# Meowuu7/equi-articulated-pose

Measured on AMD Instinct MI355X. Metric: point-clouds/sec (4096 pts, 60 anchors) fwd+bwd, higher is better.
Workload: dtype f32; 1 GPU; 8 x 4096-pt synthetic laptop clouds per GPU, 3-block inter backbone 1->64->128->512 (NN=64,K=24,A=60), forward+backward+Adam; clouds_per_gpu=8, points=4096, anchors=60

## Files before the change

### equi-articulated-pose_amd/csrc/so3_dense.hip

```cpp
#include <atomic>
#include "common.h"
#include "device_prims.h"
#include <type_traits>

namespace {

typedef unsigned long long u64;
typedef const __attribute__((address_space(4))) unsigned long long *cu64p;

constexpr int KC_BK = 32;
constexpr int KC_LIST_BYTES = 4096;

__host__ __device__ __forceinline__ void dense_kr(int d, int ks, int &k, int &r) {
    const int g = d / (16 * ks), rem = d - g * 16 * ks;
    k = rem >> 4;
    r = 16 * g + (rem & 15);
}


__device__ __forceinline__ void split2(float x0, float x1, unsigned &h, unsigned &l) {
    asm("v_cvt_pk_f16_f32 %0, %2, %3\n\t"
        "v_fma_mixlo_f16 %1, %0, -1.0, %2 op_sel:[0,0,0] op_sel_hi:[1,0,0]\n\t"
        "v_fma_mixhi_f16 %1, %0, -1.0, %3 op_sel:[1,0,0] op_sel_hi:[1,0,0]"
        : "=&v"(h), "=&v"(l) : "v"(x0), "v"(x1));
// ... 175 lines not shown
__global__ __launch_bounds__(256) void dense_rows_kernel(int n_sup, int na, int ks, int rp, int kd_pad, int rows_ld,
                                                         const float *__restrict__ s_xyz, const float *__restrict__ centre,
                                                         const int32_t *__restrict__ rows, const float *__restrict__ rk,
                                                         const float *__restrict__ row_rot, f32x4 *__restrict__ kr) {
    const int b = blockIdx.z, a = blockIdx.y, i = blockIdx.x * 256 + threadIdx.x;
    if (i >= kd_pad) return;
    f32x4 v = {1e4f, 1e4f, 1e4f, 0.f};
    if (i < ks * rp) {
        int k, r;
        dense_kr(i, ks, k, r);
        const int row = rows[(size_t)b * rows_ld + r];
        if ((unsigned)row < (unsigned)n_sup) {
            const float *kp = rk + ((size_t)a * ks + k) * 3;
            double k0 = (double)kp[0], k1 = (double)kp[1], k2 = (double)kp[2];
            if (row_rot != nullptr) {
                const float *M = row_rot + ((size_t)b * rows_ld + r) * 9;
                const double t0 = M[0] * k0 + M[1] * k1 + M[2] * k2, t1 = M[3] * k0 + M[4] * k1 + M[5] * k2, t2 = M[6] * k0 + M[7] * k1 + M[8] * k2;
                k0 = t0; k1 = t1; k2 = t2;
            }
            const double x = (double)s_xyz[((size_t)b * 3 + 0) * n_sup + row] - (double)centre[b * 4 + 0] - k0;
            const double y = (double)s_xyz[((size_t)b * 3 + 1) * n_sup + row] - (double)centre[b * 4 + 1] - k1;
            const double z = (double)s_xyz[((size_t)b * 3 + 2) * n_sup + row] - (double)centre[b * 4 + 2] - k2;
            v = (f32x4){(float)x, (float)y, (float)z, 0.f};
        }
    }
    kr[((size_t)b * na + a) * kd_pad + i] = v;
}

__global__ __launch_bounds__(256) void dense_rowmax_kernel(int m, int l, int na, int seg, long long seg_pitch4, const int32_t *__restrict__ colmap,
                                                           const f32x4 *__restrict__ T, float *__restrict__ scale, float *__restrict__ scale2) {
    __shared__ unsigned s[256][4];
    const int nq = na >> 2, G = 256 / nq, b = blockIdx.y, row = blockIdx.x, t = threadIdx.x;
    const int aq = t % nq, pg = t / nq;
    unsigned v0 = 0, v1 = 0, v2 = 0, v3 = 0;
    if (pg < G) {
        const f32x4 *src = T + ((size_t)b * m + row) * (colmap ? (size_t)1 : (size_t)(l / seg)) * seg_pitch4;
        for (int i0 = pg; i0 < l; i0 += 8 * G) {
            f32x4 q[8];
#pragma unroll
            for (int u = 0; u < 8; ++u) {
                const int i = min(i0 + u * G, l - 1), sg = i / seg;
                if (colmap != nullptr) {
                    const int ci = colmap[(size_t)b * l + i];
                    q[u] = ci >= 0 ? src[(size_t)ci * nq + aq] : (f32x4){0.f, 0.f, 0.f, 0.f};
                } else {
                    q[u] = src[(size_t)sg * seg_pitch4 + (size_t)(i - sg * seg) * nq + aq];
                }
            }
#pragma unroll
            for (int u = 0; u < 8; ++u) {
                v0 = max(v0, __float_as_uint(q[u].x) & 0x7fffffffu);
                v1 = max(v1, __float_as_uint(q[u].y) & 0x7fffffffu);
                v2 = max(v2, __float_as_uint(q[u].z) & 0x7fffffffu);
                v3 = max(v3, __float_as_uint(q[u].w) & 0x7fffffffu);
            }
        }
    }
    s[t][0] = v0; s[t][1] = v1; s[t][2] = v2; s[t][3] = v3;
    __syncthreads();
    if (t < na) {
        unsigned v = 0;
        for (int g = 0; g < G; ++g) v = max(v, s[g * nq + (t >> 2)][t & 3]);
        const float sc = pow2_scale(__uint_as_float(v));
        scale[((size_t)b * na + t) * m + row] = sc;
        scale2[((size_t)b * m + row) * na + t] = sc;
    }
}

__global__ __launch_bounds__(256) void dense_scale_kernel(long long total, int m, int na, const unsigned *__restrict__ rowmax,
                                                          float *__restrict__ scale, float *__restrict__ scale2) {
    const long long i = (long long)blockIdx.x * 256 + threadIdx.x;
    if (i >= total) return;
    const int a = (int)(i % na);
    const long long br = i / na;
    const int row = (int)(br % m);
    const long long b = br / m;
    const float sc = pow2_scale(__uint_as_float(rowmax[i]));
    scale[(b * na + a) * m + row] = sc;
    scale2[i] = sc;
}

struct SplitBn { const f32x4 *Y2; const float *coef; float slope, inv_slope; };
template <bool BN>
__global__ __launch_bounds__(256) void dense_split_kernel(int nb, int m, int l, int na, int kb_total, int seg, long long seg_pitch4, int mapped,
                                                          const int32_t *__restrict__ n_rows, const int32_t *__restrict__ colmap,
                                                          const f32x4 *__restrict__ T, const float *__restrict__ scale2,
                                                          u32x4 *__restrict__ planes, SplitBn bn) {
    const int t = threadIdx.x;
    const int mts = m >> 5;
    const int kb = (int)(blockIdx.x % (unsigned)kb_total), grp_ = (int)(blockIdx.x / (unsigned)kb_total), mt = grp_ % mts, b = grp_ / mts;
    (void)nb;
    const int nq = na >> 2, RG = 256 / nq;
    const int aq = t % nq, rr = t / nq;
    if (rr >= RG) return;
    const int MT = m >> 5, nseg = l / seg;
    if (mapped && n_rows != nullptr && 16 * kb >= ((min(n_rows[b], seg) + 15) & ~15) * nseg) return;
    for (int it0 = rr; it0 < 64; it0 += 2 * RG) {
        f32x4 q[2][8];
        f32x4 q2[BN ? 2 : 1][BN ? 8 : 1];
        int rowv[2], lanef[2];
#pragma unroll
        for (int u = 0; u < 2; ++u) {
            const int it = min(it0 + u * RG, 63);
            const int i = it & 31, kg = it >> 5, row = 32 * mt + i, l0 = 16 * kb + 8 * kg;
            rowv[u] = row; lanef[u] = i + 32 * kg;
            const size_t row_off = ((size_t)b * m + row) * (colmap ? (size_t)1 : (size_t)nseg) * seg_pitch4 + aq;
            const f32x4 *src = T + row_off;
            int sg = l0 / seg, sr = l0 - sg * seg;
            if (mapped) dense_kr(l0, nseg, sg, sr);
            if (colmap != nullptr) {
                int ci[8] = {-1, -1, -1, -1, -1, -1, -1, -1};
                if (l0 < l) {
                    const int4 c0 = *reinterpret_cast<const int4 *>(colmap + (size_t)b * l + l0), c1 = *reinterpret_cast<const int4 *>(colmap + (size_t)b * l + l0 + 4);
                    ci[0] = c0.x; ci[1] = c0.y; ci[2] = c0.z; ci[3] = c0.w; ci[4] = c1.x; ci[5] = c1.y; ci[6] = c1.z; ci[7] = c1.w;
                }
#pragma unroll
                for (int e = 0; e < 8; ++e) q[u][e] = ci[e] >= 0 ? src[(size_t)ci[e] * nq] : (f32x4){0.f, 0.f, 0.f, 0.f};
                if constexpr (BN) {
#pragma unroll
                    for (int e = 0; e < 8; ++e) q2[u][e] = ci[e] >= 0 ? bn.Y2[row_off + (size_t)ci[e] * nq] : (f32x4){0.f, 0.f, 0.f, 0.f};
                }
            } else {
#pragma unroll
                for (int e = 0; e < 8; ++e) {
                    const bool in = l0 + e < l;
                    const size_t at = (size_t)sg * seg_pitch4 + (size_t)sr * nq;
                    q[u][e] = in ? src[at] : (f32x4){0.f, 0.f, 0.f, 0.f};
                    if constexpr (BN) q2[u][e] = in ? bn.Y2[row_off + at] : (f32x4){0.f, 0.f, 0.f, 0.f};
                    if (++sr == seg) { sr = 0; ++sg; }
                }
            }
        }
        if constexpr (BN) {
#pragma unroll
            for (int u = 0; u < 2; ++u) {
                const int it = min(it0 + u * RG, 63);
                const int l0 = 16 * kb + 8 * (it >> 5);
                const float k1 = bn.coef[rowv[u]], k2 = bn.coef[m + rowv[u]], k3 = bn.coef[2 * m + rowv[u]], be = bn.coef[3 * m + rowv[u]], ig = bn.coef[4 * m + rowv[u]];
                int live = 0;
                if (colmap != nullptr) {
                    if (l0 < l) {
                        const int4 c0 = *reinterpret_cast<const int4 *>(colmap + (size_t)b * l + l0), c1 = *reinterpret_cast<const int4 *>(colmap + (size_t)b * l + l0 + 4);
                        live = (c0.x >= 0) | (c0.y >= 0) << 1 | (c0.z >= 0) << 2 | (c0.w >= 0) << 3 | (c1.x >= 0) << 4 | (c1.y >= 0) << 5 | (c1.z >= 0) << 6 | (c1.w >= 0) << 7;
                    }
                } else {
                    for (int e = 0; e < 8; ++e) live |= (l0 + e < l) << e;
                }
#pragma unroll
                for (int e = 0; e < 8; ++e)
#pragma unroll
                    for (int j = 0; j < 4; ++j) {
                        const float yv = q2[u][e][j], gv = q[u][e][j];
                        const bool pos = yv > 0.f;
                        const float gg = pos ? gv : gv * bn.slope, pre = pos ? yv : yv * bn.inv_slope;
                        const float gx = fmaf(gg, k1, -k2) - ((pre - be) * ig) * k3;
                        q[u][e][j] = ((live >> e) & 1) ? gx : 0.f;
                    }
            }
        }
#pragma unroll
        for (int u = 0; u < 2; ++u) {
            if (it0 + u * RG >= 64) break;
            const f32x4 sc = *reinterpret_cast<const f32x4 *>(scale2 + ((size_t)b * m + rowv[u]) * na + 4 * aq);
#pragma unroll
            for (int j = 0; j < 4; ++j) {
                unsigned h[4], lo[4];
#pragma unroll
                for (int e = 0; e < 4; ++e) split2(q[u][2 * e][j] * sc[j], q[u][2 * e + 1][j] * sc[j], h[e], lo[e]);
                u32x4 *dst = planes + ((((size_t)b * na + 4 * aq + j) * kb_total + kb) * MT + mt) * 128 + lanef[u];
                dst[0] = (u32x4){h[0], h[1], h[2], h[3]};
                dst[64] = (u32x4){lo[0], lo[1], lo[2], lo[3]};
            }
        }
    }
}

template <int CSTEPS>
__global__ __launch_bounds__(256) void dense_gplanes_kernel(int m, int na, int ks, int rp, int rch, int kb_total, const float *__restrict__ W3,
                                                            const float *__restrict__ Ft, const int32_t *__restrict__ n_rows,
                                                            const float *__restrict__ bound, float *__restrict__ scale, u32x4 *__restrict__ planes) {
    constexpr int C = 16 * CSTEPS, PITCH = 2 * C + 16;
    extern __shared__ __attribute__((aligned(16))) unsigned char smem[];
    __shared__ unsigned s_red[4];
    const int z = blockIdx.y, b = z / na;
    const int t = threadIdx.x, lane = t & 63, li = lane & 31, kg = lane >> 5, wave = t >> 6;
    const int rows_b = n_rows ? min((min(n_rows[b], rp) + 15) & ~15, rp) : rp;
    unsigned char *Fh = smem, *Fl = smem + (size_t)rch * PITCH;
    const int MT = m >> 5, mt = blockIdx.x * 4 + wave;
    const bool active = mt < MT;
    const int o = 32 * min(mt, MT - 1) + li;
    const float s_out = pow2_scale(bound[(size_t)z * m + o]);
    if (active && kg == 0) scale[(size_t)z * m + o] = s_out;
    for (int rc0 = 0; rc0 < rows_b; rc0 += rch) {
        const int nrows = min(rch, rows_b - rc0);
        if (rc0 > 0) __syncthreads();
        const f32x4 *src = reinterpret_cast<const f32x4 *>(Ft + ((size_t)z * rp + rc0) * C);
        const int n4 = nrows * (C / 4);
        unsigned mx = 0;
        for (int i = t; i < n4; i += 256) {
            const f32x4 v = src[i];
            mx = max(mx, max(max(__float_as_uint(v.x) & 0x7fffffffu, __float_as_uint(v.y) & 0x7fffffffu),
                             max(__float_as_uint(v.z) & 0x7fffffffu, __float_as_uint(v.w) & 0x7fffffffu)));
        }
#pragma unroll
        for (int o_ = 32; o_ > 0; o_ >>= 1) mx = max(mx, (unsigned)__shfl_xor((int)mx, o_));
        if (lane == 0) s_red[wave] = mx;
        __syncthreads();
        const float sF = pow2_scale(__uint_as_float(max(max(s_red[0], s_red[1]), max(s_red[2], s_red[3]))));
        for (int i = t; i < n4; i += 256) {
            const f32x4 v = src[i];
            const int r = i / (C / 4), c4 = i - r * (C / 4);
            unsigned h0, l0, h1, l1;
            split2(v.x * sF, v.y * sF, h0, l0);
            split2(v.z * sF, v.w * sF, h1, l1);
            *reinterpret_cast<uint2 *>(Fh + (size_t)r * PITCH + c4 * 8) = make_uint2(h0, h1);
            *reinterpret_cast<uint2 *>(Fl + (size_t)r * PITCH + c4 * 8) = make_uint2(l0, l1);
        }
        __syncthreads();
        if (!active) continue;
        const int rtiles = (nrows + 31) >> 5;
        f32x4 wn[CSTEPS][2];
        auto load_w = [&](int k) __attribute__((always_inline)) {
            const f32x4 *wrow = reinterpret_cast<const f32x4 *>(W3 + ((size_t)o * ks + k) * C) + 2 * kg;
#pragma unroll
            for (int s_ = 0; s_ < CSTEPS; ++s_) { wn[s_][0] = wrow[4 * s_]; wn[s_][1] = wrow[4 * s_ + 1]; }
        };
        load_w(0);
        for (int k = 0; k < ks; ++k) {
            f32x4 w[CSTEPS][2];
            unsigned wm = 0;
#pragma unroll
            for (int s_ = 0; s_ < CSTEPS; ++s_) {
                w[s_][0] = wn[s_][0]; w[s_][1] = wn[s_][1];
#pragma unroll
                for (int e = 0; e < 4; ++e) wm = max(wm, max(__float_as_uint(w[s_][0][e]) & 0x7fffffffu, __float_as_uint(w[s_][1][e]) & 0x7fffffffu));
            }
            if (k + 1 < ks) load_w(k + 1);
            wm = max(wm, (unsigned)__shfl_xor((int)wm, 32));
            const float sW = pow2_scale(__uint_as_float(wm));
            u32x4 Bh[CSTEPS], Bl[CSTEPS];
#pragma unroll
            for (int s_ = 0; s_ < CSTEPS; ++s_) {
                unsigned h[4], l[4];
                split2(w[s_][0].x * sW, w[s_][0].y * sW, h[0], l[0]);
                split2(w[s_][0].z * sW, w[s_][0].w * sW, h[1], l[1]);
                split2(w[s_][1].x * sW, w[s_][1].y * sW, h[2], l[2]);
                split2(w[s_][1].z * sW, w[s_][1].w * sW, h[3], l[3]);
                Bh[s_] = (u32x4){h[0], h[1], h[2], h[3]};
                Bl[s_] = (u32x4){l[0], l[1], l[2], l[3]};
            }
            const float tsc = s_out / (sF * sW);
            for (int rt = 0; rt < rtiles; ++rt) {
                f32x16 acc;
#pragma unroll
                for (int i = 0; i < 16; ++i) acc[i] = 0.f;
                const int r = min(32 * rt + li, rch - 1);
                const unsigned char *ah = Fh + (size_t)r * PITCH + 16 * kg, *al = Fl + (size_t)r * PITCH + 16 * kg;
#pragma unroll
                for (int s_ = 0; s_ < CSTEPS; ++s_) {
                    const u32x4 fh = *reinterpret_cast<const u32x4 *>(ah + 32 * s_), fl = *reinterpret_cast<const u32x4 *>(al + 32 * s_);
                    acc = __builtin_amdgcn_mfma_f32_32x32x16_f16(__builtin_bit_cast(f16x8, fh), __builtin_bit_cast(f16x8, Bh[s_]), acc, 0, 0, 0);
                    acc = __builtin_amdgcn_mfma_f32_32x32x16_f16(__builtin_bit_cast(f16x8, fh), __builtin_bit_cast(f16x8, Bl[s_]), acc, 0, 0, 0);
                    acc = __builtin_amdgcn_mfma_f32_32x32x16_f16(__builtin_bit_cast(f16x8, fl), __builtin_bit_cast(f16x8, Bh[s_]), acc, 0, 0, 0);
                }
                float av[16];
#pragma unroll
                for (int i = 0; i < 16; ++i) { av[i] = acc[i]; asm volatile("" : "+v"(av[i])); }
                const bool hi = kg != 0;
                float snd[8], rcv[8];
#pragma unroll
                for (int e = 0; e < 4; ++e) { snd[e] = hi ? av[e] : av[4 + e]; snd[4 + e] = hi ? av[8 + e] : av[12 + e]; }
#pragma unroll
                for (int e = 0; e < 8; ++e) rcv[e] = __shfl_xor(snd[e], 32);
#pragma unroll
                for (int half = 0; half < 2; ++half) {
                    float v[8];
#pragma unroll
                    for (int e = 0; e < 4; ++e) {
                        const float own = (hi ? av[4 + 8 * half + e] : av[8 * half + e]) * tsc, got = rcv[4 * half + e] * tsc;
                        v[e] = hi ? got : own;
                        v[4 + e] = hi ? own : got;
                    }
                    const int r0 = rc0 + 32 * rt + 16 * half + 8 * kg;
                    if (r0 < rc0 + nrows) {
                        unsigned h[4], l[4];
#pragma unroll
                        for (int e = 0; e < 4; ++e) split2(v[2 * e], v[2 * e + 1], h[e], l[e]);
                        const int kb = (r0 >> 4) * ks + k;
                        u32x4 *dst = planes + (((size_t)z * kb_total + kb) * MT + mt) * 128 + li + 32 * kg;
                        dst[0] = (u32x4){h[0], h[1], h[2], h[3]};
                        dst[64] = (u32x4){l[0], l[1], l[2], l[3]};
                    }
                }
            }
        }
    }
}

__global__ __launch_bounds__(256) void dense_untranspose_kernel(int nb, int o_total, int p, int na, int p_dst, const int32_t *__restrict__ map,
                                                                const int32_t *__restrict__ pivot_pos,
                                                                const float *__restrict__ yt, float *__restrict__ y,
                                                                float *__restrict__ psum, float *__restrict__ psq,
                                                                const float *__restrict__ bn_scale = nullptr, const float *__restrict__ bn_shift = nullptr,
                                                                float slope = 1.f) {
    extern __shared__ float tile[];
    __shared__ float red[2][256];
    const int chunks = (p + 63) >> 6, t = threadIdx.x;
    const int p0 = (int)(blockIdx.x % (unsigned)chunks) * 64, grp_ = (int)(blockIdx.x / (unsigned)chunks), o = grp_ % o_total, b = grp_ / o_total;
    const int nchunk_x = chunks, nb_z = nb;
    const int np = min(64, p - p0);
    const float pivot = psum ? yt[(size_t)o * p + (pivot_pos ? *pivot_pos : 0)] : 0.f;
    float s = 0.f, q = 0.f;
    for (int i = t; i < na * 64; i += 256) {
        const int a = i >> 6, pp = i & 63;
        if (pp < np) {
            const float v = yt[(((size_t)b * na + a) * o_total + o) * p + p0 + pp];
            tile[a * 65 + pp] = v;
            if (psum != nullptr && (map == nullptr || map[(size_t)b * p + p0 + pp] >= 0)) {
                const float d = v - pivot;
                s += d; q = fmaf(d, d, q);
            }
        }
    }
    red[0][t] = s; red[1][t] = q;
    __syncthreads();
    const int nq = na >> 2;
    float *rows_y = y + ((size_t)b * o_total + o) * (size_t)(map ? p_dst : p) * na;
    for (int i = t; i < np * nq; i += 256) {
        const int pp = i / nq, a4 = i - pp * nq;
        const int q = map ? map[(size_t)b * p + p0 + pp] : p0 + pp;
        if (map != nullptr && (unsigned)q >= (unsigned)p_dst) continue;
        const float *src = tile + (4 * a4) * 65 + pp;
        f32x4 v = {src[0], src[65], src[130], src[195]};
        if (bn_scale != nullptr) {
            const float sc = bn_scale[o], sh = bn_shift[o];
#pragma unroll
            for (int e = 0; e < 4; ++e) { const float u = fmaf(v[e], sc, sh); v[e] = u > 0.f ? u : u * slope; }
        }
        *reinterpret_cast<f32x4 *>(rows_y + (size_t)q * na + 4 * a4) = v;
    }
    if (psum == nullptr) return;
    for (int h = 128; h > 0; h >>= 1) {
        if (t < h) { red[0][t] += red[0][t + h]; red[1][t] += red[1][t + h]; }
        __syncthreads();
    }
    if (t == 0) {
        const size_t at = ((size_t)o * nb_z + b) * nchunk_x + (p0 >> 6);
        psum[at] = red[0][0]; psq[at] = red[1][0];
    }
}

__global__ __launch_bounds__(256) void dense_zero_tail_kernel(int rows_ok, int na, int rp, long long ldz, const int32_t *__restrict__ n_rows,
                                                              float *__restrict__ z) {
    const int b = blockIdx.y, row = blockIdx.x;
    const int r0 = (min(n_rows[b], rp) + 15) & ~15, tail = rp - r0;
    if (tail <= 0) return;
    float *dst = z + ((long long)b * rows_ok + row) * ldz;
    for (int e = threadIdx.x; e < na * tail; e += 256) {
        const int a = e / tail;
        dst[(long long)a * rp + r0 + (e - a * tail)] = 0.f;
    }
}

struct KcArgs {
    int MT, N, KS, na, zcount;
    int tiles_m, blocks_n, mask_tiles;
    const u32x4 *A;
    const float *scale;
    const f32x4 *strT; long long strB, strA;
    const f32x4 *colT; long long colB, colA;
    const unsigned *mask;
    float neg_inv_sigma;
    const int32_t *n_rows; int ks, trim;
    float *C; long long cB, cA, ldm; int rp; long long kstride;
    int row_slots;
    const int32_t *steps;
};

template <int MI>
__global__ __launch_bounds__(256, MI == 4 ? 2 : 1) void kc_gemm_kernel(KcArgs g) {
    static_assert(MI == 8 || MI == 4, "the DMA piece schedule below: 8 or 4 KB of the stored operand per wave and k-step");
    constexpr unsigned WB = MI * 1024u;
    constexpr unsigned SUB_A = MI * 2048u;
    constexpr unsigned STR_OFF = 2 * SUB_A;
    constexpr unsigned BIT_OFF = STR_OFF + 1024u;
    constexpr unsigned STAGE = BIT_OFF + 1024u;
    extern __shared__ __attribute__((aligned(16))) unsigned char smem[];

    const int per_z = g.tiles_m * g.blocks_n;
    int id = blockIdx.x, z, local;
    {
        const int groups = g.zcount / 8 * 8;
        if (id < groups * per_z) {
            const int xcd = id & 7, slot = id >> 3;
            z = (slot / per_z) * 8 + xcd;
            local = slot % per_z;
        } else {
            const int r = id - groups * per_z;
            z = groups + r / per_z;
            local = r % per_z;
        }
    }
    const int bm = local % g.tiles_m, bn = local / g.tiles_m;
    const int b = z / g.na, a = z - b * g.na;
    const int used = (g.trim == 1 || g.trim == 2) ? ((min(g.n_rows[b], g.row_slots) + 15) & ~15) * g.ks : 0;
    const int N = g.trim == 1 ? min(g.N, used) : g.N;
    if (256 * bn >= N) return;
    const int32_t *lstG = g.steps ? g.steps + ((size_t)b * g.blocks_n + bn) * (size_t)(g.KS + 1) : nullptr;
    const int KS = lstG ? __builtin_amdgcn_readfirstlane(lstG[0]) : (g.trim == 2 ? max(min(g.KS, used / KC_BK), 1) : g.KS);
    int *lstL = reinterpret_cast<int *>(smem + 4 * STAGE);
    if (lstG != nullptr) {
        for (int i = threadIdx.x; i < KS; i += 256) lstL[i] = lstG[1 + i];
        __syncthreads();
    }
    auto step_at = [&](int i) __attribute__((always_inline)) { return lstG ? __builtin_amdgcn_readfirstlane(lstL[i]) : i; };

    const int t = threadIdx.x, lane = t & 63, li = lane & 31, kg = lane >> 5;
    const int wave = __builtin_amdgcn_readfirstlane(t >> 6);
    const int wt = bn * 4 + wave;
    const bool active = 64 * wt < N;

    const f32x4 *colz = g.colT + b * g.colB + a * g.colA;
    f32x4 cc[2];
#pragma unroll
    for (int j = 0; j < 2; ++j) cc[j] = colz[min(64 * wt + 32 * j + li, N - 1)];
    const float nis = g.neg_inv_sigma;

    const unsigned char *Aw = reinterpret_cast<const unsigned char *>(g.A) + ((size_t)z * 2 * g.KS * g.MT + (size_t)bm * MI) * 2048u
                              + (size_t)(wave >> 1) * ((size_t)g.MT * 2048u) + (size_t)(wave & 1) * WB;
    const size_t step_bytes = (size_t)g.MT * 4096u;
    const unsigned char *strw = reinterpret_cast<const unsigned char *>(g.strT + b * g.strB + a * g.strA) + (size_t)(wave & 1) * 256u;
// ... 199 lines not shown
           (o % 128) == 0;
}
}

extern "C" int eap_so3_dense_supported(int p, int na, int ks, int rp, int o) { return dense_shape_ok(p, na, ks, rp, o, MEMB_WORDS_WIDE); }

extern "C" int eap_so3_dense_max_rows(void) { return DENSE_MAX_ROWS; }

extern "C" int64_t eap_so3_dense_mask_words(int b, int p, int ks, int rp, int dir) {
    const int n = dir ? p : ks * rp, kd = dir ? ceil_to(ks * rp, KC_BK) : p;
    const int wtiles = 4 * ((n + 255) / 256), steps = kd / KC_BK;
    return ((int64_t)b * wtiles * steps * 64 + 1) / 2;
}

namespace {
template <int W>
int dense_member(int b, int p, int n_sup, int nn, int rp, int rows_ld, const int32_t *idx, const int32_t *rows, const int32_t *n_rows, int32_t *slot_of,
                 uint32_t *memb, int32_t *flags, eap_stream_t stream) {
    if (b <= 0 || p <= 0) return 0;
    if (rp <= 0 || rp > 32 * W) return eap::bad_arg(W == MEMB_WORDS ? "so3_dense_member: 0 < rp <= 512" : "so3_dense_member_wide: 0 < rp <= 1024");
    hipStream_t s = eap::S(stream);
    if (int e = eap::hip_fail(hipMemsetAsync(slot_of, 0xff, sizeof(int32_t) * (size_t)b * n_sup, s), "so3_dense_member memset")) return e;
    if (int e = eap::hip_fail(hipMemsetAsync(flags, 0, sizeof(int32_t) * (size_t)b, s), "so3_dense_member memset")) return e;
    if (int e = eap::run_kernel("so3_dense_member", dense_slots_kernel, eap::cdiv(rp, 256), b, 1, dim3(256), 0, s, n_sup, rp, rows_ld, rows, n_rows, slot_of)) return e;
    return eap::run_kernel("so3_dense_member", dense_member_kernel<W>, eap::cdiv(p, 256), b, 1, dim3(256), 0, s, p, n_sup, nn, rp, idx, slot_of, memb, flags);
}

template <int W>
int dense_masks(int b, int p, int ks, int rp, int dir, const uint32_t *memb, uint64_t *mask, eap_stream_t stream) {
    if (b <= 0) return 0;
    if (!dense_shape_ok(p, 4, ks, rp, 256, W)) return eap::bad_arg("so3_dense_masks: shape not taken");
    const int n = dir ? p : ks * rp, kd = dir ? ceil_to(ks * rp, KC_BK) : p;
    const int wtiles = 4 * ((n + 255) / 256), steps = kd / KC_BK;
    return eap::run_kernel("so3_dense_masks", dense_mask_kernel<W>, eap::cdiv((long long)wtiles * steps, 4), b, 1, dim3(256), 0, eap::S(stream), p, ks, rp, dir, wtiles, steps,
                           memb, reinterpret_cast<unsigned *>(mask));
}
}

extern "C" int eap_so3_dense_member(int b, int p, int n_sup, int nn, int rp, int rows_ld, const int32_t *idx, const int32_t *rows,
                                    const int32_t *n_rows, int32_t *slot_of, uint32_t *memb, int32_t *flags, eap_stream_t stream) {
    return dense_member<MEMB_WORDS>(b, p, n_sup, nn, rp, rows_ld, idx, rows, n_rows, slot_of, memb, flags, stream);
}

extern "C" int eap_so3_dense_member_wide(int b, int p, int n_sup, int nn, int rp, int rows_ld, const int32_t *idx, const int32_t *rows,
                                         const int32_t *n_rows, int32_t *slot_of, uint32_t *memb, int32_t *flags, eap_stream_t stream) {
    return dense_member<MEMB_WORDS_WIDE>(b, p, n_sup, nn, rp, rows_ld, idx, rows, n_rows, slot_of, memb, flags, stream);
}

extern "C" int eap_so3_dense_masks(int b, int p, int ks, int rp, int dir, const uint32_t *memb, uint64_t *mask, eap_stream_t stream) {
    return dense_masks<MEMB_WORDS>(b, p, ks, rp, dir, memb, mask, stream);
}

extern "C" int eap_so3_dense_masks_wide(int b, int p, int ks, int rp, int dir, const uint32_t *memb, uint64_t *mask, eap_stream_t stream) {
    return dense_masks<MEMB_WORDS_WIDE>(b, p, ks, rp, dir, memb, mask, stream);
}

extern "C" int eap_so3_dense_tables_f32(int b, int p, int n_sup, int na, int ks, int rp, int rows_ld, float sigma, const float *q_xyz,
                                        const float *s_xyz, const int32_t *rows, const float *rk, const float *row_rot, float *centre, float *pt,
                                        float *kr, eap_stream_t stream) {
    if (b <= 0) return 0;
    if (!(sigma > 0.f)) return eap::bad_arg("so3_dense_tables: sigma > 0");
    hipStream_t s = eap::S(stream);
    const int p_pad = ceil_to(p, KC_BK), kd_pad = ceil_to(ks * rp, KC_BK);
    if (int e = eap::run_kernel("so3_dense_tables", dense_centre_kernel, b, 1, 1, dim3(256), 0, s, n_sup, s_xyz, centre)) return e;
    if (int e = eap::run_kernel("so3_dense_tables", dense_points_kernel, eap::cdiv(p_pad, 256), b, 1, dim3(256), 0, s, p, p_pad, q_xyz, centre,
                                reinterpret_cast<f32x4 *>(pt)))
        return e;
    return eap::run_kernel("so3_dense_tables", dense_rows_kernel, eap::cdiv(kd_pad, 256), na, b, dim3(256), 0, s, n_sup, na, ks, rp, kd_pad, rows_ld,
                           s_xyz, centre, rows, rk, row_rot, reinterpret_cast<f32x4 *>(kr));
}

extern "C" int eap_so3_dense_split_f32(int b, int m, int l, int na, int seg, int64_t seg_pitch, int mapped, const int32_t *n_rows, const uint32_t *rowmax,
                                       const int32_t *colmap, const float *src, float *scale, void *planes, eap_stream_t stream) {
    if (b <= 0) return 0;
    if (colmap != nullptr) {
        if (mapped || seg_pitch <= 0 || (l & 7) != 0 || (reinterpret_cast<uintptr_t>(colmap) & 15) != 0)
            return eap::bad_arg("so3_dense_split: a column map (16-byte aligned, a multiple of 8 columns) comes with the source row pitch and without the dense-index mapping");
        seg = l;
    }
    if (seg <= 0) { seg = l; seg_pitch = (int64_t)l * na; }
    if ((m % 32) != 0 || (na % 4) != 0 || na > 64 || (reinterpret_cast<uintptr_t>(src) & 15) || l % seg != 0 ||
        (seg_pitch & 3) != 0 || (colmap == nullptr && seg_pitch < (int64_t)seg * na) || (mapped && ((seg % 16) != 0 || ((l / seg) % 2) != 0)))
        return eap::bad_arg("so3_dense_split: m % 32, na % 4, na <= 64, 16-byte aligned source, whole segments of a 16-byte aligned pitch (mapped: seg % 16, an even number of segments)");
    hipStream_t s = eap::S(stream);
    const int kb_total = ceil_to(l, KC_BK) / 16;
    float *scale2 = scale + (size_t)b * na * m;
    const int e = rowmax != nullptr
                      ? eap::run_kernel("so3_dense_split", dense_scale_kernel, eap::cdiv((long long)b * m * na, 256), 1, 1, dim3(256), 0, s, (long long)b * m * na, m, na, rowmax, scale, scale2)
                      : eap::run_kernel("so3_dense_split", dense_rowmax_kernel, m, b, 1, dim3(256), 0, s, m, l, na, seg, (long long)(seg_pitch / 4), colmap,
                                        reinterpret_cast<const f32x4 *>(src), scale, scale2);
    if (e) return e;
    return eap::run_kernel("so3_dense_split", dense_split_kernel<false>, (long long)kb_total * (m / 32) * b, 1, 1, dim3(256), 0, s, b, m, l, na, kb_total, seg, (long long)(seg_pitch / 4),
                           mapped ? 1 : 0, n_rows, colmap, reinterpret_cast<const f32x4 *>(src), scale2, reinterpret_cast<u32x4 *>(planes), SplitBn{nullptr, nullptr, 1.f, 1.f});
}

extern "C" int eap_so3_dense_split_bn_f32(int b, int m, int l, int l_src, int na, const uint32_t *rowbound, const int32_t *colmap, const float *grad,
                                          const float *act, const float *coef, float slope, float *scale, void *planes, eap_stream_t stream) {
    if (b <= 0) return 0;
    if (colmap == nullptr && l != l_src) return eap::bad_arg("so3_dense_split_bn: without a column map l = l_src");
    if ((m % 32) != 0 || (na % 4) != 0 || na > 64 || ((reinterpret_cast<uintptr_t>(grad) | reinterpret_cast<uintptr_t>(act)) & 15) ||
        (colmap != nullptr && ((l & 7) != 0 || (reinterpret_cast<uintptr_t>(colmap) & 15) != 0)) || rowbound == nullptr || coef == nullptr || !(slope > 0.f))
        return eap::bad_arg("so3_dense_split_bn: m % 32, na % 4, na <= 64, 16-byte aligned sources, a bound per row, a positive slope (column map: 16-byte aligned, l % 8)");
    hipStream_t s = eap::S(stream);
    const int kb_total = ceil_to(l, KC_BK) / 16;
    float *scale2 = scale + (size_t)b * na * m;
    if (int e = eap::run_kernel("so3_dense_split_bn", dense_scale_kernel, eap::cdiv((long long)b * m * na, 256), 1, 1, dim3(256), 0, s, (long long)b * m * na, m, na, rowbound, scale,
                                scale2))
        return e;
    const int seg = colmap ? l : l_src;
    return eap::run_kernel("so3_dense_split_bn", dense_split_kernel<true>, (long long)kb_total * (m / 32) * b, 1, 1, dim3(256), 0, s, b, m, l, na, kb_total, seg,
                           (long long)l_src * na / 4, 0, nullptr, colmap, reinterpret_cast<const f32x4 *>(grad), scale2, reinterpret_cast<u32x4 *>(planes),
                           SplitBn{reinterpret_cast<const f32x4 *>(act), coef, slope, 1.0f / slope});
}

extern "C" int eap_so3_dense_untranspose_bnact_f32(int b, int o, int p, int na, int p_dst, const int32_t *map, const float *yt, const float *bn_scale,
                                                   const float *bn_shift, float slope, float *y, eap_stream_t stream) {
    if (b <= 0) return 0;
    if (bn_scale == nullptr || bn_shift == nullptr || (map != nullptr && p_dst <= 0) || (map == nullptr && p_dst != p))
        return eap::bad_arg("so3_dense_untranspose_bnact: scale and shift per channel; p_dst = p without a map");
    return eap::run_kernel("so3_dense_untranspose_bnact", dense_untranspose_kernel, (long long)eap::cdiv(p, 64) * o * b, 1, 1, dim3(256), sizeof(float) * (size_t)na * 65, eap::S(stream), b, o, p, na,
                           p_dst, map, nullptr, yt, y, nullptr, nullptr, bn_scale, bn_shift, slope);
}

extern "C" int eap_so3_dense_gplanes_supported(int o, int c, int na, int ks, int rp) {
    return (o % 32) == 0 && (c == 64 || c == 128) && na > 0 && ks > 0 && (ks % 2) == 0 && rp > 0 && (rp % 16) == 0;
}

extern "C" int eap_so3_dense_gplanes_f32(int b, int o, int c, int na, int ks, int rp, const float *W3, const float *Ft, const int32_t *n_rows,
                                         const float *bound, float *scale, void *planes, eap_stream_t stream) {
    if (b <= 0) return 0;
    if (!eap_so3_dense_gplanes_supported(o, c, na, ks, rp) ||
        ((reinterpret_cast<uintptr_t>(W3) | reinterpret_cast<uintptr_t>(Ft) | reinterpret_cast<uintptr_t>(planes)) & 15) != 0)
        return eap::bad_arg("so3_dense_gplanes: shape not taken (eap_so3_dense_gplanes_supported), 16-byte aligned operands");
    const int kb_total = ceil_to(ks * rp, KC_BK) / 16;
    const int fit = (int)((84u * 1024u) / ((size_t)(2 * c + 16) * 2)) / 16 * 16;
    const int rch = min(rp, max(fit, 32));
    const size_t shmem = (size_t)rch * (2 * c + 16) * 2;
    return eap::run_kernel("so3_dense_gplanes", c == 128 ? dense_gplanes_kernel<8> : dense_gplanes_kernel<4>, eap::cdiv(o / 32, 4), (long long)b * na, 1, dim3(256), shmem,
                           eap::S(stream), o, na, ks, rp, rch, kb_total, W3, Ft, n_rows, bound, scale, reinterpret_cast<u32x4 *>(planes));
}

extern "C" int eap_so3_dense_product_steps_f32(int dir, int b, int o, int p, int na, int ks, int rp, int64_t ldz, float sigma, const int32_t *n_rows,
                                               const void *planes, const float *scale, const float *pt, const float *kr, const uint64_t *mask,
                                               const int32_t *steps, float *out, eap_stream_t stream) {
    if (b <= 0) return 0;
    if (!eap_so3_dense_supported(p, na, ks, rp, o)) return eap::bad_arg("so3_dense_product: shape not taken (eap_so3_dense_supported)");
    const int p_pad = ceil_to(p, KC_BK), kd_pad = ceil_to(ks * rp, KC_BK);
    KcArgs g;
    g.MT = o / 32; g.na = na; g.zcount = b * na; g.row_slots = rp;
    g.N = dir ? p : ks * rp;
    g.KS = (dir ? kd_pad : p) / KC_BK;
    const bool wide = (o % 256) == 0;
    g.tiles_m = wide ? o / 256 : o / 128;
    g.blocks_n = (g.N + 255) / 256;
    g.mask_tiles = 4 * g.blocks_n;
    g.A = reinterpret_cast<const u32x4 *>(planes);
    g.scale = scale;
    const f32x4 *ptT = reinterpret_cast<const f32x4 *>(pt), *krT = reinterpret_cast<const f32x4 *>(kr);
    if (dir == 0) {
        g.strT = ptT; g.strB = p_pad; g.strA = 0;
        g.colT = krT; g.colB = (long long)na * kd_pad; g.colA = kd_pad;
        if (ldz < (int64_t)na * rp) return eap::bad_arg("so3_dense_product: ldz < na rp");
        g.cB = (long long)o * ks * ldz; g.cA = rp; g.ldm = (long long)ks * ldz; g.rp = rp; g.kstride = ldz;
    } else {
        g.strT = krT; g.strB = (long long)na * kd_pad; g.strA = kd_pad;
        g.colT = ptT; g.colB = p_pad; g.colA = 0;
        g.cB = (long long)na * o * p; g.cA = (long long)o * p; g.ldm = p; g.rp = p; g.kstride = 0;
    }
    g.mask = reinterpret_cast<const unsigned *>(mask);
    g.steps = (steps != nullptr && g.KS <= KC_LIST_BYTES / 4) ? steps : nullptr;
    g.C = out;
    g.neg_inv_sigma = -1.0f / sigma;
    g.n_rows = n_rows; g.ks = ks; g.trim = dir ? 2 : 1;
    if (n_rows == nullptr) g.trim = dir ? 0 : 3;
    if (dir == 0 && n_rows != nullptr) {
        if (int e = eap::run_kernel("so3_dense zero tail", dense_zero_tail_kernel, (long long)o * ks, b, 1, dim3(256), 0, eap::S(stream), o * ks, na, rp, (long long)ldz, n_rows, out))
            return e;
    }
    return wide ? kc_launch<8>(g, eap::S(stream)) : kc_launch<4>(g, eap::S(stream));
}

extern "C" int eap_so3_dense_product_f32(int dir, int b, int o, int p, int na, int ks, int rp, int64_t ldz, float sigma, const int32_t *n_rows,
                                         const void *planes, const float *scale, const float *pt, const float *kr, const uint64_t *mask, float *out, eap_stream_t stream) {
    return eap_so3_dense_product_steps_f32(dir, b, o, p, na, ks, rp, ldz, sigma, n_rows, planes, scale, pt, kr, mask, nullptr, out, stream);
}

extern "C" int eap_so3_dense_point_keys(int b, int p, const uint32_t *memb, int32_t *keys, eap_stream_t stream) {
    if (b <= 0 || p <= 0) return 0;
    const long long total = (long long)b * p;
    return eap::run_kernel("so3_dense_point_keys", dense_keys_kernel<MEMB_WORDS>, eap::cdiv(total, 256), 1, 1, dim3(256), 0, eap::S(stream), total, memb, keys);
}

extern "C" int eap_so3_dense_point_keys_wide(int b, int p, const uint32_t *memb, int64_t *keys, eap_stream_t stream) {
    if (b <= 0 || p <= 0) return 0;
    const long long total = (long long)b * p;
    return eap::run_kernel("so3_dense_point_keys_wide", dense_keys_kernel<MEMB_WORDS_WIDE>, eap::cdiv(total, 256), 1, 1, dim3(256), 0, eap::S(stream), total, memb, keys);
}

extern "C" int64_t eap_so3_dense_steps_words(int b, int p, int ks, int rp, int dir) {
    const int n = dir ? p : ks * rp, kd = dir ? ceil_to(ks * rp, KC_BK) : p;
    return (int64_t)b * ((n + 255) / 256) * (kd / KC_BK + 1);
}

namespace {
int dense_steps(int words, int b, int p, int ks, int rp, int dir, int skip, const int32_t *n_rows, const uint64_t *mask, int32_t *steps, eap_stream_t stream) {
    if (b <= 0) return 0;
    if (!dense_shape_ok(p, 4, ks, rp, 256, words)) return eap::bad_arg("so3_dense_steps: shape not taken");
    const int n = dir ? p : ks * rp, kd = dir ? ceil_to(ks * rp, KC_BK) : p;
    const int blocks_n = (n + 255) / 256, KS = kd / KC_BK;
    if ((size_t)KS * sizeof(int) > 48 * 1024) return eap::bad_arg("so3_dense_steps: more than 12288 k-steps");
    return eap::run_kernel("so3_dense_steps", dense_steps_kernel, blocks_n, b, 1, dim3(256), sizeof(int) * (size_t)KS, eap::S(stream), KS, blocks_n, 4 * blocks_n, dir, ks, rp, skip,
                           n_rows, reinterpret_cast<const unsigned *>(mask), steps);
}
}

extern "C" int eap_so3_dense_steps(int b, int p, int ks, int rp, int dir, int skip, const int32_t *n_rows, const uint64_t *mask, int32_t *steps,
                                   eap_stream_t stream) {
    return dense_steps(MEMB_WORDS, b, p, ks, rp, dir, skip, n_rows, mask, steps, stream);
}

extern "C" int eap_so3_dense_steps_wide(int b, int p, int ks, int rp, int dir, int skip, const int32_t *n_rows, const uint64_t *mask, int32_t *steps,
                                        eap_stream_t stream) {
    return dense_steps(MEMB_WORDS_WIDE, b, p, ks, rp, dir, skip, n_rows, mask, steps, stream);
}

extern "C" int eap_so3_dense_untranspose_f32(int b, int o, int p, int na, const float *yt, float *y, float *psum, float *psq, eap_stream_t stream) {
    if (b <= 0) return 0;
    return eap::run_kernel("so3_dense_untranspose", dense_untranspose_kernel, (long long)eap::cdiv(p, 64) * o * b, 1, 1, dim3(256), sizeof(float) * (size_t)na * 65, eap::S(stream), b, o, p, na,
                           p, nullptr, nullptr, yt, y, psum, psum ? psq : nullptr, nullptr, nullptr, 1.f);
}

extern "C" int eap_so3_dense_untranspose_map_f32(int b, int o, int p, int na, int p_dst, const int32_t *map, const float *yt, float *y,
                                                 eap_stream_t stream) {
    if (b <= 0) return 0;
    if (map == nullptr || p_dst <= 0) return eap::bad_arg("so3_dense_untranspose_map: a map, p_dst > 0");
    return eap::run_kernel("so3_dense_untranspose_map", dense_untranspose_kernel, (long long)eap::cdiv(p, 64) * o * b, 1, 1, dim3(256), sizeof(float) * (size_t)na * 65, eap::S(stream), b, o, p, na,
                           p_dst, map, nullptr, yt, y, nullptr, nullptr, nullptr, nullptr, 1.f);
}

extern "C" int eap_so3_dense_untranspose_map_stats_f32(int b, int o, int p, int na, int p_dst, const int32_t *map, const int32_t *pivot_pos, const float *yt,
                                                       float *y, float *psum, float *psq, eap_stream_t stream) {
    if (b <= 0) return 0;
    if (map == nullptr || pivot_pos == nullptr || p_dst <= 0 || psum == nullptr || psq == nullptr)
        return eap::bad_arg("so3_dense_untranspose_map_stats: a map, the pivot column, both partial arrays");
    return eap::run_kernel("so3_dense_untranspose_map_stats", dense_untranspose_kernel, (long long)eap::cdiv(p, 64) * o * b, 1, 1, dim3(256), sizeof(float) * (size_t)na * 65, eap::S(stream), b, o, p, na,
                           p_dst, map, pivot_pos, yt, y, psum, psq, nullptr, nullptr, 1.f);
}
```

Measured before the change: 156.3 point-clouds/sec.

## Stage split planes in LDS and add tiled untranspose kernel for non-stats paths

The split kernel now gives each block one of the two k-groups (grid doubled). It writes its fp16 hi/lo planes into a rotated shared-memory image and then stores them to global memory in coalesced order, instead of making strided per-lane stores. Column offsets and masks are computed once per block and masked lanes are zeroed with bitmasks. A new 128-point tiled untranspose kernel with swizzled LDS, vectorised loads and block reordering replaces the old one for the plain, map and BN-activation variants. The cost is more LDS per block (na*1KB), a waves-per-EU cap, and new argument checks.

```diff
diff --git a/equi-articulated-pose_amd/csrc/so3_dense.hip b/equi-articulated-pose_amd/csrc/so3_dense.hip
--- a/equi-articulated-pose_amd/csrc/so3_dense.hip
+++ b/equi-articulated-pose_amd/csrc/so3_dense.hip
@@ -281,70 +281,66 @@
 
 struct SplitBn { const f32x4 *Y2; const float *coef; float slope, inv_slope; };
 template <bool BN>
-__global__ __launch_bounds__(256) void dense_split_kernel(int nb, int m, int l, int na, int kb_total, int seg, long long seg_pitch4, int mapped,
+__global__ __launch_bounds__(256) __attribute__((amdgpu_waves_per_eu(2, 2))) void dense_split_kernel(int m, int l, int na, int kb_total, int seg, long long seg_pitch4, int mapped,
                                                           const int32_t *__restrict__ n_rows, const int32_t *__restrict__ colmap,
                                                           const f32x4 *__restrict__ T, const float *__restrict__ scale2,
                                                           u32x4 *__restrict__ planes, SplitBn bn) {
+    extern __shared__ u32x4 image[];
     const int t = threadIdx.x;
-    const int mts = m >> 5;
-    const int kb = (int)(blockIdx.x % (unsigned)kb_total), grp_ = (int)(blockIdx.x / (unsigned)kb_total), mt = grp_ % mts, b = grp_ / mts;
-    (void)nb;
+    const int MT = m >> 5;
+    const unsigned blk = blockIdx.x >> 1;
+    const int kg = (int)(blockIdx.x & 1u), kb = (int)(blk % (unsigned)kb_total), grp_ = (int)(blk / (unsigned)kb_total), mt = grp_ % MT, b = grp_ / MT;
     const int nq = na >> 2, RG = 256 / nq;
     const int aq = t % nq, rr = t / nq;
-    if (rr >= RG) return;
-    const int MT = m >> 5, nseg = l / seg;
+    const int nseg = l / seg;
     if (mapped && n_rows != nullptr && 16 * kb >= ((min(n_rows[b], seg) + 15) & ~15) * nseg) return;
-    for (int it0 = rr; it0 < 64; it0 += 2 * RG) {
+    const int l0 = 16 * kb + 8 * kg;
+    unsigned at[8], keep[8];
+    int live = 0;
+    if (colmap != nullptr) {
+        int ci[8] = {-1, -1, -1, -1, -1, -1, -1, -1};
+        if (l0 < l) {
+            const int4 c0 = *reinterpret_cast<const int4 *>(colmap + (size_t)b * l + l0), c1 = *reinterpret_cast<const int4 *>(colmap + (size_t)b * l + l0 + 4);
+            ci[0] = c0.x; ci[1] = c0.y; ci[2] = c0.z; ci[3] = c0.w; ci[4] = c1.x; ci[5] = c1.y; ci[6] = c1.z; ci[7] = c1.w;
+        }
+#pragma unroll
+        for (int e = 0; e < 8; ++e) { keep[e] = ci[e] >= 0 ? ~0u : 0u; at[e] = (unsigned)max(ci[e], 0) * (unsigned)nq; live |= (int)(keep[e] & 1u) << e; }
+    } else {
+        int sg = l0 / seg, sr = l0 - sg * seg;
+        if (mapped) dense_kr(l0, nseg, sg, sr);
+#pragma unroll
+        for (int e = 0; e < 8; ++e) {
+            keep[e] = l0 + e < l ? ~0u : 0u;
+            at[e] = keep[e] ? (unsigned)sg * (unsigned)seg_pitch4 + (unsigned)sr * (unsigned)nq : 0u;
+            live |= (int)(keep[e] & 1u) << e;
+            if (++sr == seg) { sr = 0; ++sg; }
+        }
+#pragma unroll
+        for (int e = 1; e < 8; ++e) at[e] = keep[e] ? at[e] : at[0];
+    }
+    if (live == 0)
+        for (int i = t; i < 64 * na; i += 256) image[i] = (u32x4){0u, 0u, 0u, 0u};
+    for (int it0 = rr; it0 < 32 && rr < RG && live != 0; it0 += 2 * RG) {
         f32x4 q[2][8];
         f32x4 q2[BN ? 2 : 1][BN ? 8 : 1];
-        int rowv[2], lanef[2];
+        int rowv[2];
 #pragma unroll
         for (int u = 0; u < 2; ++u) {
-            const int it = min(it0 + u * RG, 63);
-            const int i = it & 31, kg = it >> 5, row = 32 * mt + i, l0 = 16 * kb + 8 * kg;
-            rowv[u] = row; lanef[u] = i + 32 * kg;
+            const int row = 32 * mt + min(it0 + u * RG, 31);
+            rowv[u] = row;
             const size_t row_off = ((size_t)b * m + row) * (colmap ? (size_t)1 : (size_t)nseg) * seg_pitch4 + aq;
-            const f32x4 *src = T + row_off;
-            int sg = l0 / seg, sr = l0 - sg * seg;
-            if (mapped) dense_kr(l0, nseg, sg, sr);
-            if (colmap != nullptr) {
-                int ci[8] = {-1, -1, -1, -1, -1, -1, -1, -1};
-                if (l0 < l) {
-                    const int4 c0 = *reinterpret_cast<const int4 *>(colmap + (size_t)b * l + l0), c1 = *reinterpret_cast<const int4 *>(colmap + (size_t)b * l + l0 + 4);
-                    ci[0] = c0.x; ci[1] = c0.y; ci[2] = c0.z; ci[3] = c0.w; ci[4] = c1.x; ci[5] = c1.y; ci[6] = c1.z; ci[7] = c1.w;
-                }
-#pragma unroll
-                for (int e = 0; e < 8; ++e) q[u][e] = ci[e] >= 0 ? src[(size_t)ci[e] * nq] : (f32x4){0.f, 0.f, 0.f, 0.f};
-                if constexpr (BN) {
-#pragma unroll
-                    for (int e = 0; e < 8; ++e) q2[u][e] = ci[e] >= 0 ? bn.Y2[row_off + (size_t)ci[e] * nq] : (f32x4){0.f, 0.f, 0.f, 0.f};
-                }
-            } else {
-#pragma unroll
-                for (int e = 0; e < 8; ++e) {
-                    const bool in = l0 + e < l;
-                    const size_t at = (size_t)sg * seg_pitch4 + (size_t)sr * nq;
-                    q[u][e] = in ? src[at] : (f32x4){0.f, 0.f, 0.f, 0.f};
-                    if constexpr (BN) q2[u][e] = in ? bn.Y2[row_off + at] : (f32x4){0.f, 0.f, 0.f, 0.f};
-                    if (++sr == seg) { sr = 0; ++sg; }
-                }
-            }
-        }
+#pragma unroll
+            for (int e = 0; e < 8; ++e) q[u][e] = T[row_off + at[e]];
+            if constexpr (BN) {
+#pragma unroll
+                for (int e = 0; e < 8; ++e) q2[u][e] = bn.Y2[row_off + at[e]];
+            }
+        }
+        __builtin_amdgcn_sched_barrier(0);
         if constexpr (BN) {
 #pragma unroll
             for (int u = 0; u < 2; ++u) {
-                const int it = min(it0 + u * RG, 63);
-                const int l0 = 16 * kb + 8 * (it >> 5);
                 const float k1 = bn.coef[rowv[u]], k2 = bn.coef[m + rowv[u]], k3 = bn.coef[2 * m + rowv[u]], be = bn.coef[3 * m + rowv[u]], ig = bn.coef[4 * m + rowv[u]];
-                int live = 0;
-                if (colmap != nullptr) {
-                    if (l0 < l) {
-                        const int4 c0 = *reinterpret_cast<const int4 *>(colmap + (size_t)b * l + l0), c1 = *reinterpret_cast<const int4 *>(colmap + (size_t)b * l + l0 + 4);
-                        live = (c0.x >= 0) | (c0.y >= 0) << 1 | (c0.z >= 0) << 2 | (c0.w >= 0) << 3 | (c1.x >= 0) << 4 | (c1.y >= 0) << 5 | (c1.z >= 0) << 6 | (c1.w >= 0) << 7;
-                    }
-                } else {
-                    for (int e = 0; e < 8; ++e) live |= (l0 + e < l) << e;
-                }
 #pragma unroll
                 for (int e = 0; e < 8; ++e)
 #pragma unroll
@@ -353,24 +349,38 @@
                         const bool pos = yv > 0.f;
                         const float gg = pos ? gv : gv * bn.slope, pre = pos ? yv : yv * bn.inv_slope;
                         const float gx = fmaf(gg, k1, -k2) - ((pre - be) * ig) * k3;
-                        q[u][e][j] = ((live >> e) & 1) ? gx : 0.f;
+                        q[u][e][j] = __uint_as_float(__float_as_uint(gx) & keep[e]);
                     }
             }
+        } else if (live != 255) {
+#pragma unroll
+            for (int u = 0; u < 2; ++u)
+#pragma unroll
+                for (int e = 0; e < 8; ++e)
+#pragma unroll
+                    for (int j = 0; j < 4; ++j) q[u][e][j] = __uint_as_float(__float_as_uint(q[u][e][j]) & keep[e]);
         }
 #pragma unroll
         for (int u = 0; u < 2; ++u) {
-            if (it0 + u * RG >= 64) break;
+            const int i = it0 + u * RG;
+            if (i >= 32) break;
             const f32x4 sc = *reinterpret_cast<const f32x4 *>(scale2 + ((size_t)b * m + rowv[u]) * na + 4 * aq);
+            u32x4 *dst = image + 256 * aq + ((i + aq) & 31);
 #pragma unroll
             for (int j = 0; j < 4; ++j) {
                 unsigned h[4], lo[4];
 #pragma unroll
                 for (int e = 0; e < 4; ++e) split2(q[u][2 * e][j] * sc[j], q[u][2 * e + 1][j] * sc[j], h[e], lo[e]);
-                u32x4 *dst = planes + ((((size_t)b * na + 4 * aq + j) * kb_total + kb) * MT + mt) * 128 + lanef[u];
-                dst[0] = (u32x4){h[0], h[1], h[2], h[3]};
-                dst[64] = (u32x4){lo[0], lo[1], lo[2], lo[3]};
-            }
-        }
+                dst[64 * j] = (u32x4){h[0], h[1], h[2], h[3]};
+                dst[64 * j + 32] = (u32x4){lo[0], lo[1], lo[2], lo[3]};
+            }
+        }
+    }
+    __syncthreads();
+    const int w = t >> 6, pl = (t >> 5) & 1, i = t & 31;
+    for (int k = 0; k < nq; ++k) {
+        const int a = 4 * k + w;
+        planes[((((size_t)b * na + a) * kb_total + kb) * MT + mt) * 128 + 64 * pl + 32 * kg + i] = image[64 * a + 32 * pl + ((i + k) & 31)];
     }
 }
 
@@ -499,9 +509,7 @@
 __global__ __launch_bounds__(256) void dense_untranspose_kernel(int nb, int o_total, int p, int na, int p_dst, const int32_t *__restrict__ map,
                                                                 const int32_t *__restrict__ pivot_pos,
                                                                 const float *__restrict__ yt, float *__restrict__ y,
-                                                                float *__restrict__ psum, float *__restrict__ psq,
-                                                                const float *__restrict__ bn_scale = nullptr, const float *__restrict__ bn_shift = nullptr,
-                                                                float slope = 1.f) {
+                                                                float *__restrict__ psum, float *__restrict__ psq) {
     extern __shared__ float tile[];
     __shared__ float red[2][256];
     const int chunks = (p + 63) >> 6, t = threadIdx.x;
@@ -530,12 +538,7 @@
         const int q = map ? map[(size_t)b * p + p0 + pp] : p0 + pp;
         if (map != nullptr && (unsigned)q >= (unsigned)p_dst) continue;
         const float *src = tile + (4 * a4) * 65 + pp;
-        f32x4 v = {src[0], src[65], src[130], src[195]};
-        if (bn_scale != nullptr) {
-            const float sc = bn_scale[o], sh = bn_shift[o];
-#pragma unroll
-            for (int e = 0; e < 4; ++e) { const float u = fmaf(v[e], sc, sh); v[e] = u > 0.f ? u : u * slope; }
-        }
+        const f32x4 v = {src[0], src[65], src[130], src[195]};
         *reinterpret_cast<f32x4 *>(rows_y + (size_t)q * na + 4 * a4) = v;
     }
     if (psum == nullptr) return;
@@ -546,6 +549,68 @@
     if (t == 0) {
         const size_t at = ((size_t)o * nb_z + b) * nchunk_x + (p0 >> 6);
         psum[at] = red[0][0]; psq[at] = red[1][0];
+    }
+}
+
+constexpr int UT_PTS = 128;
+__global__ __launch_bounds__(256, 5) void dense_untranspose_tile_kernel(int o_total, int p, int na, int p_dst, const int32_t *__restrict__ map,
+                                                                     const float *__restrict__ yt, float *__restrict__ y,
+                                                                     const float *__restrict__ bn_scale, const float *__restrict__ bn_shift, float slope) {
+    constexpr int UT_LD = UT_PTS / 16;
+    extern __shared__ float tile[];
+    __shared__ int dst_row[UT_PTS];
+    const int chunks = (p + UT_PTS - 1) / UT_PTS, t = threadIdx.x;
+    unsigned bid = blockIdx.x;
+    if (const unsigned n8 = gridDim.x / 8u; bid < 8u * n8) bid = (bid % 8u) * n8 + bid / 8u;
+    const int p0 = (int)(bid % (unsigned)chunks) * UT_PTS, grp_ = (int)(bid / (unsigned)chunks), o = grp_ % o_total, b = grp_ / o_total;
+    const int np = min(UT_PTS, p - p0);
+    if (t < UT_PTS) dst_row[t] = t >= np ? -1 : map ? map[(size_t)b * p + p0 + t] : p0 + t;
+    const size_t a_pitch = (size_t)o_total * p;
+    const float *src = yt + ((size_t)b * na * o_total + o) * p + p0;
+    if ((p & 3) == 0) {
+        f32x4 v[UT_LD];
+#pragma unroll
+        for (int k = 0; k < UT_LD; ++k) {
+            const int i = t + 256 * k, a = i / (UT_PTS / 4), c = 4 * (i % (UT_PTS / 4));
+            if (a < na && c < np) v[k] = *reinterpret_cast<const f32x4 *>(src + (size_t)a * a_pitch + c);
+        }
+#pragma unroll
+        for (int k = 0; k < UT_LD; ++k) {
+            const int i = t + 256 * k, a = i / (UT_PTS / 4), c = 4 * (i % (UT_PTS / 4));
+            if (a < na && c < np) *reinterpret_cast<f32x4 *>(tile + a * UT_PTS + ((c + 4 * ((a >> 2) & 7)) & (UT_PTS - 1))) = v[k];
+        }
+    } else {
+        for (int i = t; i < na * UT_PTS; i += 256) {
+            const int a = i / UT_PTS, c = i % UT_PTS;
+            if (c < np) tile[a * UT_PTS + ((c + 4 * ((a >> 2) & 7)) & (UT_PTS - 1))] = src[(size_t)a * a_pitch + c];
+        }
+    }
+    __syncthreads();
+    const int nq = na >> 2, RG = 256 / nq, a4 = t % nq, rr = t / nq;
+    if (rr >= RG) return;
+    const int rows_dst = map ? p_dst : p, rot = 4 * (a4 & 7);
+    const float *quad = tile + (4 * a4) * UT_PTS;
+    float *rows_y = y + ((size_t)b * o_total + o) * (size_t)rows_dst * na + 4 * a4;
+    float sc = 1.f, sh = 0.f;
+    if (bn_scale != nullptr) { sc = bn_scale[o]; sh = bn_shift[o]; }
+    for (int pp0 = rr; pp0 < np; pp0 += 4 * RG) {
+        f32x4 v[4];
+        int q[4];
+#pragma unroll
+        for (int u = 0; u < 4; ++u) {
+            const int pp = min(pp0 + u * RG, UT_PTS - 1), c = (pp + rot) & (UT_PTS - 1);
+            q[u] = pp0 + u * RG < np ? dst_row[pp] : -1;
+            v[u] = (f32x4){quad[c], quad[UT_PTS + c], quad[2 * UT_PTS + c], quad[3 * UT_PTS + c]};
+        }
+#pragma unroll
+        for (int u = 0; u < 4; ++u) {
+            if ((unsigned)q[u] >= (unsigned)rows_dst) continue;
+            if (bn_scale != nullptr) {
+#pragma unroll
+                for (int e = 0; e < 4; ++e) { const float w = fmaf(v[u][e], sc, sh); v[u][e] = w > 0.f ? w : w * slope; }
+            }
+            *reinterpret_cast<f32x4 *>(rows_y + (size_t)q[u] * na) = v[u];
+        }
     }
 }
 
@@ -911,6 +976,7 @@
     if ((m % 32) != 0 || (na % 4) != 0 || na > 64 || (reinterpret_cast<uintptr_t>(src) & 15) || l % seg != 0 ||
         (seg_pitch & 3) != 0 || (colmap == nullptr && seg_pitch < (int64_t)seg * na) || (mapped && ((seg % 16) != 0 || ((l / seg) % 2) != 0)))
         return eap::bad_arg("so3_dense_split: m % 32, na % 4, na <= 64, 16-byte aligned source, whole segments of a 16-byte aligned pitch (mapped: seg % 16, an even number of segments)");
+    if ((colmap ? (int64_t)1 : (int64_t)(l / seg)) * (seg_pitch / 4) > 0x7fffffffLL) return eap::bad_arg("so3_dense_split: a source row of at most 2^31 16-byte pieces");
     hipStream_t s = eap::S(stream);
     const int kb_total = ceil_to(l, KC_BK) / 16;
     float *scale2 = scale + (size_t)b * na * m;
@@ -919,7 +985,7 @@
                       : eap::run_kernel("so3_dense_split", dense_rowmax_kernel, m, b, 1, dim3(256), 0, s, m, l, na, seg, (long long)(seg_pitch / 4), colmap,
                                         reinterpret_cast<const f32x4 *>(src), scale, scale2);
     if (e) return e;
-    return eap::run_kernel("so3_dense_split", dense_split_kernel<false>, (long long)kb_total * (m / 32) * b, 1, 1, dim3(256), 0, s, b, m, l, na, kb_total, seg, (long long)(seg_pitch / 4),
+    return eap::run_kernel("so3_dense_split", dense_split_kernel<false>, (long long)kb_total * (m / 32) * b * 2, 1, 1, dim3(256), (size_t)na * 1024, s, m, l, na, kb_total, seg, (long long)(seg_pitch / 4),
                            mapped ? 1 : 0, n_rows, colmap, reinterpret_cast<const f32x4 *>(src), scale2, reinterpret_cast<u32x4 *>(planes), SplitBn{nullptr, nullptr, 1.f, 1.f});
 }
 
@@ -930,6 +996,7 @@
     if ((m % 32) != 0 || (na % 4) != 0 || na > 64 || ((reinterpret_cast<uintptr_t>(grad) | reinterpret_cast<uintptr_t>(act)) & 15) ||
         (colmap != nullptr && ((l & 7) != 0 || (reinterpret_cast<uintptr_t>(colmap) & 15) != 0)) || rowbound == nullptr || coef == nullptr || !(slope > 0.f))
         return eap::bad_arg("so3_dense_split_bn: m % 32, na % 4, na <= 64, 16-byte aligned sources, a bound per row, a positive slope (column map: 16-byte aligned, l % 8)");
+    if ((int64_t)l_src * na / 4 > 0x7fffffffLL) return eap::bad_arg("so3_dense_split_bn: a source row of at most 2^31 16-byte pieces");
     hipStream_t s = eap::S(stream);
     const int kb_total = ceil_to(l, KC_BK) / 16;
     float *scale2 = scale + (size_t)b * na * m;
@@ -937,9 +1004,30 @@
                                 scale2))
         return e;
     const int seg = colmap ? l : l_src;
-    return eap::run_kernel("so3_dense_split_bn", dense_split_kernel<true>, (long long)kb_total * (m / 32) * b, 1, 1, dim3(256), 0, s, b, m, l, na, kb_total, seg,
+    return eap::run_kernel("so3_dense_split_bn", dense_split_kernel<true>, (long long)kb_total * (m / 32) * b * 2, 1, 1, dim3(256), (size_t)na * 1024, s, m, l, na, kb_total, seg,
                            (long long)l_src * na / 4, 0, nullptr, colmap, reinterpret_cast<const f32x4 *>(grad), scale2, reinterpret_cast<u32x4 *>(planes),
                            SplitBn{reinterpret_cast<const f32x4 *>(act), coef, slope, 1.0f / slope});
+}
+
+namespace {
+int untranspose_args(const char *what, int o, int p, int na, const float *yt, const float *y) {
+    char buf[256];
+    const char *why = nullptr;
+    if (o <= 0 || p <= 0) why = "o > 0 and p > 0";
+    else if (na <= 0 || (na % 4) != 0) why = "na % 4 == 0 (rows of Y are stored as 16-byte pieces)";
+    else if (na > 64) why = "na <= 64 (the tile of a block)";
+    else if (yt == nullptr || (reinterpret_cast<uintptr_t>(yt) & 15) != 0) why = "yt 16-byte aligned";
+    else if (y == nullptr || (reinterpret_cast<uintptr_t>(y) & 15) != 0) why = "y 16-byte aligned";
+    if (why == nullptr) return 0;
+    snprintf(buf, sizeof(buf), "%s: %s", what, why);
+    return eap::bad_arg(buf);
+}
+
+int untranspose_tile(const char *what, int b, int o, int p, int na, int p_dst, const int32_t *map, const float *yt, float *y, const float *bn_scale,
+                     const float *bn_shift, float slope, eap_stream_t stream) {
+    return eap::run_kernel(what, dense_untranspose_tile_kernel, (long long)eap::cdiv(p, UT_PTS) * o * b, 1, 1, dim3(256), sizeof(float) * (size_t)na * UT_PTS,
+                           eap::S(stream), o, p, na, p_dst, map, yt, y, bn_scale, bn_shift, slope);
+}
 }
 
 extern "C" int eap_so3_dense_untranspose_bnact_f32(int b, int o, int p, int na, int p_dst, const int32_t *map, const float *yt, const float *bn_scale,
@@ -947,8 +1035,8 @@
     if (b <= 0) return 0;
     if (bn_scale == nullptr || bn_shift == nullptr || (map != nullptr && p_dst <= 0) || (map == nullptr && p_dst != p))
         return eap::bad_arg("so3_dense_untranspose_bnact: scale and shift per channel; p_dst = p without a map");
-    return eap::run_kernel("so3_dense_untranspose_bnact", dense_untranspose_kernel, (long long)eap::cdiv(p, 64) * o * b, 1, 1, dim3(256), sizeof(float) * (size_t)na * 65, eap::S(stream), b, o, p, na,
-                           p_dst, map, nullptr, yt, y, nullptr, nullptr, bn_scale, bn_shift, slope);
+    if (int e = untranspose_args("so3_dense_untranspose_bnact", o, p, na, yt, y)) return e;
+    return untranspose_tile("so3_dense_untranspose_bnact", b, o, p, na, p_dst, map, yt, y, bn_scale, bn_shift, slope, stream);
 }
 
 extern "C" int eap_so3_dense_gplanes_supported(int o, int c, int na, int ks, int rp) {
@@ -1055,16 +1143,19 @@
 
 extern "C" int eap_so3_dense_untranspose_f32(int b, int o, int p, int na, const float *yt, float *y, float *psum, float *psq, eap_stream_t stream) {
     if (b <= 0) return 0;
+    if (int e = untranspose_args("so3_dense_untranspose", o, p, na, yt, y)) return e;
+    if (psum == nullptr) return untranspose_tile("so3_dense_untranspose", b, o, p, na, p, nullptr, yt, y, nullptr, nullptr, 1.f, stream);
+    if (psq == nullptr) return eap::bad_arg("so3_dense_untranspose: both partial arrays or neither");
     return eap::run_kernel("so3_dense_untranspose", dense_untranspose_kernel, (long long)eap::cdiv(p, 64) * o * b, 1, 1, dim3(256), sizeof(float) * (size_t)na * 65, eap::S(stream), b, o, p, na,
-                           p, nullptr, nullptr, yt, y, psum, psum ? psq : nullptr, nullptr, nullptr, 1.f);
+                           p, nullptr, nullptr, yt, y, psum, psq);
 }
 
 extern "C" int eap_so3_dense_untranspose_map_f32(int b, int o, int p, int na, int p_dst, const int32_t *map, const float *yt, float *y,
                                                  eap_stream_t stream) {
     if (b <= 0) return 0;
     if (map == nullptr || p_dst <= 0) return eap::bad_arg("so3_dense_untranspose_map: a map, p_dst > 0");
-    return eap::run_kernel("so3_dense_untranspose_map", dense_untranspose_kernel, (long long)eap::cdiv(p, 64) * o * b, 1, 1, dim3(256), sizeof(float) * (size_t)na * 65, eap::S(stream), b, o, p, na,
-                           p_dst, map, nullptr, yt, y, nullptr, nullptr, nullptr, nullptr, 1.f);
+    if (int e = untranspose_args("so3_dense_untranspose_map", o, p, na, yt, y)) return e;
+    return untranspose_tile("so3_dense_untranspose_map", b, o, p, na, p_dst, map, yt, y, nullptr, nullptr, 1.f, stream);
 }
 
 extern "C" int eap_so3_dense_untranspose_map_stats_f32(int b, int o, int p, int na, int p_dst, const int32_t *map, const int32_t *pivot_pos, const float *yt,
@@ -1072,6 +1163,7 @@
     if (b <= 0) return 0;
     if (map == nullptr || pivot_pos == nullptr || p_dst <= 0 || psum == nullptr || psq == nullptr)
         return eap::bad_arg("so3_dense_untranspose_map_stats: a map, the pivot column, both partial arrays");
+    if (int e = untranspose_args("so3_dense_untranspose_map_stats", o, p, na, yt, y)) return e;
     return eap::run_kernel("so3_dense_untranspose_map_stats", dense_untranspose_kernel, (long long)eap::cdiv(p, 64) * o * b, 1, 1, dim3(256), sizeof(float) * (size_t)na * 65, eap::S(stream), b, o, p, na,
-                           p_dst, map, pivot_pos, yt, y, psum, psq, nullptr, nullptr, 1.f);
-}
+                           p_dst, map, pivot_pos, yt, y, psum, psq);
+}
```

Measured after the change: 161.2 point-clouds/sec (median of 6 runs). 1.03x the previous value.
